# DiamondLightSource/volume-segmantics

Hardware: AMD Instinct MI355X
Metric: slices/sec fwd+bwd U-Net/ResNet-34 256x256 bf16 batch 32 (training step incl. loss, AdamW) (higher is better)
Workload: dtype bf16; 1 GPU; configs[1]: synthetic 256^3-style 1-ch slices, 2-class, U-Net/ResNet-34, batch 32 per GPU, train step (fwd + DiceLoss + bwd + AdamW + OneCycleLR); global_batch=32, slice=256x256, parallelism=dp1, master_weights=fp32

## Files before the change

volume-segmantics_amd/csrc/conv_common.h:

```cpp
#pragma once
#include <type_traits>

#include "common.h"

template <typename T> struct CT;
template <> struct CT<bf16_t> { static constexpr int CK = 32, EPS = 8; };
template <> struct CT<f16_t> { static constexpr int CK = 32, EPS = 8; };
template <> struct CT<float> { static constexpr int CK = 16, EPS = 4; };

template <typename T>
__device__ __forceinline__ float4 ld4_roundtrip(const float (&v)[4]) {
    if constexpr (sizeof(T) == 2) {
        const float a[4] = {v[0], v[1], v[2], v[3]};
        T t[4];
        for (int i = 0; i < 4; ++i) Elem<T>::st(t + i, a[i]);
        return make_float4(Elem<T>::ld(t), Elem<T>::ld(t + 1), Elem<T>::ld(t + 2), Elem<T>::ld(t + 3));
    } else
        return make_float4(v[0], v[1], v[2], v[3]);
}

template <typename T>
__device__ __forceinline__ void mma16(f32x4& acc, const uint4& a, const uint4& b) {
    if constexpr (std::is_same<T, f16_t>::value) {
        acc = __builtin_amdgcn_mfma_f32_16x16x32_f16(__builtin_bit_cast(f16x8, a), __builtin_bit_cast(f16x8, b), acc, 0, 0, 0);
    } else if constexpr (sizeof(T) == 2) {
        acc = __builtin_amdgcn_mfma_f32_16x16x32_bf16(__builtin_bit_cast(bf16x8, a), __builtin_bit_cast(bf16x8, b),
                                                      acc, 0, 0, 0);
    } else {
        const float4 fa = __builtin_bit_cast(float4, a), fb = __builtin_bit_cast(float4, b);
        acc = __builtin_amdgcn_mfma_f32_16x16x4f32(fa.x, fb.x, acc, 0, 0, 0);
        acc = __builtin_amdgcn_mfma_f32_16x16x4f32(fa.y, fb.y, acc, 0, 0, 0);
        acc = __builtin_amdgcn_mfma_f32_16x16x4f32(fa.z, fb.z, acc, 0, 0, 0);
        acc = __builtin_amdgcn_mfma_f32_16x16x4f32(fa.w, fb.w, acc, 0, 0, 0);
    }
}


template <typename T, int BN, int PT, int NW = 4>
__device__ __forceinline__ void conv_epilogue(const ConvParams& p, int tw_shift, int out_nchw, int n, int h0, int w0, int n0,
                                              int tile, f32x4 (&acc)[PT][BN / 16], char* smem) {
    constexpr int NJ = BN / 16;
    const int tid = threadIdx.x, lane = tid & 63, wave = tid >> 6;
    const int lq = lane >> 4, lr = lane & 15;
    const int TW = 1 << tw_shift;
    struct { int tw_shift, out_nchw; } g{tw_shift, out_nchw};
    const bool ragged = (p.Cout & 3) != 0 || g.out_nchw;
    if (p.stats_partial || p.stats_bins) {
        float* red = reinterpret_cast<float*>(smem);
        __syncthreads();
#pragma unroll
        for (int j = 0; j < NJ; ++j) {
            float s1[4] = {0.f, 0.f, 0.f, 0.f}, s2[4] = {0.f, 0.f, 0.f, 0.f};
#pragma unroll
            for (int i = 0; i < PT; ++i) {
                const int pl = wave * (PT * 16) + i * 16 + lr;
                const bool ok = h0 + (pl >> g.tw_shift) < p.Hout && w0 + (pl & (TW - 1)) < p.Wout;
#pragma unroll
                for (int r = 0; r < 4; ++r) {
                    const float x = ok ? acc[i][j][r] : 0.f;
                    s1[r] += x; s2[r] += x * x;
                }
            }
#pragma unroll
            for (int r = 0; r < 4; ++r) {
#pragma unroll
                for (int o = 1; o < 16; o <<= 1) { s1[r] += __shfl_xor(s1[r], o, 64); s2[r] += __shfl_xor(s2[r], o, 64); }
            }
            if (lr == 0) {
#pragma unroll
                for (int r = 0; r < 4; ++r) {
                    red[(wave * 2 + 0) * BN + j * 16 + lq * 4 + r] = s1[r];
                    red[(wave * 2 + 1) * BN + j * 16 + lq * 4 + r] = s2[r];
                }
            }
        }
        __syncthreads();
        if (tid < 2 * BN) {
            const int k = tid / BN, cc = tid % BN;
            if (n0 + cc < p.Cout) {
                float a = 0.f;
#pragma unroll
                for (int w = 0; w < NW; ++w) a += red[(w * 2 + k) * BN + cc];
                if (p.stats_bins)
                    atomicAdd(p.stats_bins + ((size_t)(tile & (p.stats_nb - 1)) * 2 + k) * p.Cout + n0 + cc,
                              (unsigned long long)__double2ll_rn((double)a * (k ? kStatScale2 : kStatScale1)));
                else
                    p.stats_partial[((size_t)tile * 2 + k) * p.Cout + n0 + cc] = a;
            }
        }
    }
    if (p.bz) {
        float* red = reinterpret_cast<float*>(smem);
        __syncthreads();
        typename Raw4<T>::type rv[PT][NJ], zq[PT][NJ], yq[PT][NJ];
        size_t off[PT][NJ];
        bool live[PT][NJ];
#pragma unroll
        for (int j = 0; j < NJ; ++j) {
            const int c = n0 + j * 16 + lq * 4;
#pragma unroll
            for (int i = 0; i < PT; ++i) {
                const int pl = wave * (PT * 16) + i * 16 + lr;
                const int ho = h0 + (pl >> g.tw_shift), wo = w0 + (pl & (TW - 1));
                live[i][j] = ho < p.Hout && wo < p.Wout && c < p.Cout;
                off[i][j] = (((size_t)n * p.Hout + ho) * p.Wout + wo) * p.Cout + c;
                rv[i][j] = zq[i][j] = yq[i][j] = typename Raw4<T>::type{};
                if (live[i][j]) {
                    if (p.residual) rv[i][j] = ld4raw((const T*)p.residual + off[i][j]);
                    zq[i][j] = ld4raw((const T*)p.bz + off[i][j]);
                    if (p.brelu && p.by) yq[i][j] = ld4raw((const T*)p.by + off[i][j]);
                }
            }
        }
#pragma unroll
        for (int j = 0; j < NJ; ++j) {
            const int c = n0 + j * 16 + lq * 4;
            float s1[4] = {0.f, 0.f, 0.f, 0.f}, s2[4] = {0.f, 0.f, 0.f, 0.f};
            float mu[4] = {0.f, 0.f, 0.f, 0.f}, is[4] = {0.f, 0.f, 0.f, 0.f}, ga[4] = {0.f, 0.f, 0.f, 0.f}, be[4] = {0.f, 0.f, 0.f, 0.f};
            if (c < p.Cout) {
                const float4 m4 = *reinterpret_cast<const float4*>(p.bmean + c), i4 = *reinterpret_cast<const float4*>(p.binvstd + c);
                mu[0] = m4.x; mu[1] = m4.y; mu[2] = m4.z; mu[3] = m4.w;
                is[0] = i4.x; is[1] = i4.y; is[2] = i4.z; is[3] = i4.w;
                if (p.brelu && !p.by) {
                    const float4 g4 = *reinterpret_cast<const float4*>(p.bgamma + c), b4 = *reinterpret_cast<const float4*>(p.bbeta + c);
                    ga[0] = is[0] * g4.x; ga[1] = is[1] * g4.y; ga[2] = is[2] * g4.z; ga[3] = is[3] * g4.w;
                    be[0] = b4.x; be[1] = b4.y; be[2] = b4.z; be[3] = b4.w;
                }
            }
#pragma unroll
            for (int i = 0; i < PT; ++i) {
                if (!live[i][j]) continue;
                const float4 r4 = unpack4(rv[i][j]), z4 = unpack4(zq[i][j]), y4 = unpack4(yq[i][j]);
                float v[4] = {acc[i][j][0] + r4.x, acc[i][j][1] + r4.y, acc[i][j][2] + r4.z, acc[i][j][3] + r4.w};
                const float zv[4] = {z4.x, z4.y, z4.z, z4.w};
                if (p.brelu) {
                    if (p.by) {
                        v[0] = y4.x > 0.f ? v[0] : 0.f; v[1] = y4.y > 0.f ? v[1] : 0.f;
                        v[2] = y4.z > 0.f ? v[2] : 0.f; v[3] = y4.w > 0.f ? v[3] : 0.f;
                    } else {
#pragma unroll
                        for (int r = 0; r < 4; ++r) v[r] = ((zv[r] - mu[r]) * ga[r] + be[r]) > 0.f ? v[r] : 0.f;
                    }
                }
                st4((T*)p.out + off[i][j], make_float4(v[0], v[1], v[2], v[3]));
                const float4 gq = ld4_roundtrip<T>(v);
                const float gv[4] = {gq.x, gq.y, gq.z, gq.w};
#pragma unroll
                for (int r = 0; r < 4; ++r) { s1[r] += gv[r]; s2[r] += gv[r] * (zv[r] - mu[r]) * is[r]; }
            }
#pragma unroll
            for (int r = 0; r < 4; ++r) {
#pragma unroll
                for (int o = 1; o < 16; o <<= 1) { s1[r] += __shfl_xor(s1[r], o, 64); s2[r] += __shfl_xor(s2[r], o, 64); }
            }
            if (lr == 0) {
#pragma unroll
                for (int r = 0; r < 4; ++r) {
                    red[(wave * 2 + 0) * BN + j * 16 + lq * 4 + r] = s1[r];
                    red[(wave * 2 + 1) * BN + j * 16 + lq * 4 + r] = s2[r];
                }
            }
        }
        __syncthreads();
        if (tid < 2 * BN) {
            const int k = tid / BN, cc = tid % BN;
            if (n0 + cc < p.Cout) {
                float a = 0.f;
#pragma unroll
                for (int w = 0; w < NW; ++w) a += red[(w * 2 + k) * BN + cc];
                p.bstats_partial[((size_t)tile * 2 + k) * p.Cout + n0 + cc] = a;
            }
        }
        return;
    }
    const int pool_c = p.pool0 ? (p.out1 ? p.split_c : p.Cout) : 0;
#pragma unroll
    for (int j = 0; j < NJ; ++j) {
        const int c = n0 + j * 16 + lq * 4;
        if (PT >= 2 && c < pool_c) {
            if constexpr (PT >= 2) {
#pragma unroll
                for (int ip = 0; ip < PT / 2; ++ip) {
                    float v[4];
#pragma unroll
                    for (int r = 0; r < 4; ++r) {
                        v[r] = acc[2 * ip][j][r] + acc[2 * ip + 1][j][r];
                        v[r] += __shfl_xor(v[r], 1, 64);
                    }
                    const int ho = h0 + wave * PT + 2 * ip, wo = w0 + lr;
                    if ((lr & 1) == 0 && ho < p.Hout && wo < p.Wout && c < p.Cout) {
                        const size_t o = (((size_t)n * (p.Hout >> 1) + (ho >> 1)) * (p.Wout >> 1) + (wo >> 1)) * pool_c + c;
                        st4((T*)p.out + o, make_float4(v[0], v[1], v[2], v[3]));
                    }
                }
            }
            continue;
        }
#pragma unroll
        for (int i = 0; i < PT; ++i) {
            const int pl = wave * (PT * 16) + i * 16 + lr;
            const int ho = h0 + (pl >> g.tw_shift), wo = w0 + (pl & (TW - 1));
            if (ho >= p.Hout || wo >= p.Wout || c >= p.Cout) continue;
            const size_t pix = ((size_t)n * p.Hout + ho) * p.Wout + wo;
            float v[4] = {acc[i][j][0], acc[i][j][1], acc[i][j][2], acc[i][j][3]};
            if (!ragged) {
                if (p.scale) {
                    const float4 sc = *reinterpret_cast<const float4*>(p.scale + c);
                    const float4 sh = *reinterpret_cast<const float4*>(p.shift + c);
                    v[0] = v[0] * sc.x + sh.x; v[1] = v[1] * sc.y + sh.y; v[2] = v[2] * sc.z + sh.z; v[3] = v[3] * sc.w + sh.w;
                } else if (p.shift) {
                    const float4 sh = *reinterpret_cast<const float4*>(p.shift + c);
                    v[0] += sh.x; v[1] += sh.y; v[2] += sh.z; v[3] += sh.w;
                }
                char* dst = (char*)p.out;
                int cd = c, cstride = p.Cout;
                if (p.out1) {
                    if (c >= p.split_c) { dst = (char*)p.out1; cd = c - p.split_c; cstride = p.Cout - p.split_c; }
                    else cstride = p.split_c;
                }
                const size_t o = pix * cstride + cd;
                if (p.residual && dst == (char*)p.out) {
                    const float4 rv = ld4((const T*)p.residual + o);
                    v[0] += rv.x; v[1] += rv.y; v[2] += rv.z; v[3] += rv.w;
                }
                if (p.relu == 1) { v[0] = fmaxf(v[0], 0.f); v[1] = fmaxf(v[1], 0.f); v[2] = fmaxf(v[2], 0.f); v[3] = fmaxf(v[3], 0.f); }
                else if (p.relu == 2) {
#pragma unroll
                    for (int r = 0; r < 4; ++r) v[r] = v[r] / (1.f + __expf(-v[r]));
                }
                if (p.out_f32) st4((float*)dst + o, make_float4(v[0], v[1], v[2], v[3]));
                else st4((T*)dst + o, make_float4(v[0], v[1], v[2], v[3]));
            } else {
                const int nv = min(4, p.Cout - c);
                for (int r = 0; r < nv; ++r) {
                    float x = v[r];
                    if (p.scale) x = x * p.scale[c + r] + p.shift[c + r];
                    else if (p.shift) x += p.shift[c + r];
                    if (p.residual) x += Elem<T>::ld((const T*)p.residual + pix * p.Cout + c + r);
                    if (p.relu == 1) x = fmaxf(x, 0.f);
                    else if (p.relu == 2) x = x / (1.f + __expf(-x));
                    if (g.out_nchw) ((float*)p.out)[(((size_t)n * p.Cout + c + r) * p.Hout + ho) * p.Wout + wo] = x;
                    else if (p.out_f32) ((float*)p.out)[pix * p.Cout + c + r] = x;
                    else Elem<T>::st((T*)p.out + pix * p.Cout + c + r, x);
                }
            }
        }
    }
}
```

volume-segmantics_amd/csrc/conv_ring.h:

```cpp
#pragma once
#include "conv_common.h"

namespace ring {

constexpr int kRow = 64;

__device__ __forceinline__ u32x4 make_srd(const void* base, unsigned bytes) {
    const unsigned long long a = (unsigned long long)base;
    u32x4 d;
    d.x = __builtin_amdgcn_readfirstlane((unsigned)a);
    d.y = __builtin_amdgcn_readfirstlane((unsigned)(a >> 32) & 0xffffu);
    d.z = __builtin_amdgcn_readfirstlane(bytes);
    d.w = 0x00020000u;
    return d;
}
template <int IMM>
__device__ __forceinline__ void dma16(const u32x4& srd, unsigned lds_base, int voff, int soff) {
    unsigned keep;
    asm volatile("s_mov_b32 %0, m0\n\ts_add_u32 m0, %1, %5\n\ts_nop 0\n\tbuffer_load_dwordx4 %2, %3, %4 offen lds\n\ts_mov_b32 m0, %0"
                 : "=&s"(keep) : "s"(lds_base), "v"(voff), "s"(srd), "s"(soff), "n"(IMM) : "memory", "scc");
}

template <typename A>
__device__ __forceinline__ A reload_first_kernarg() {
#if defined(__HIP_DEVICE_COMPILE__)
    const __attribute__((address_space(4))) A* pk = (const __attribute__((address_space(4))) A*)__builtin_amdgcn_kernarg_segment_ptr();
    asm volatile("" : "+s"(pk));
    return *pk;
#else
    return A{};
#endif
}

struct Geom {
    int tiles_h, tiles_w;
    int groups, ctiles;
    int xcs, xgn, ctl;
    unsigned ct_magic, ti_magic, tw_magic;
    int out_nchw;
    unsigned long long* probe;
};

constexpr int cdivc(int a, int b) { return (a + b - 1) / b; }
constexpr int minc(int a, int b) { return a < b ? a : b; }
template <int V> struct IC { static constexpr int value = V; };
template <int LO, int HI, typename F>
__device__ __forceinline__ void static_for(F&& f) {
    if constexpr (LO < HI) { f(IC<LO>{}); static_for<LO + 1, HI>(f); }
}

template <int BN, int PT, int NW, int TWS, int IMGS, int WPS, int PIN, bool NLOAD = false>
__global__ __launch_bounds__(NW * 64, WPS) void conv_ring_kernel(ConvParams p, Geom g) {
    typedef bf16_t T;
    constexpr int NT = NW * 64, NJ = BN / 16, BM = NW * PT * 16, TW = 1 << TWS, TH = BM / IMGS / TW;
    constexpr int PH = TH + 2, PW = TW + 2, PP = PH * PW, P = IMGS * PP;
    constexpr int PIT = cdivc(P * 4, NT);
    constexpr int WROWS = 9 * BN, TS = NT / 4 / BN;
    static_assert((NT / 4) % BN == 0, "cout tile must divide the rows of a piece pass");
    constexpr int WIT = cdivc(WROWS * 4, NT);
    constexpr int PATCH_B = PIT * NT * 16, WGT_B = WIT * NT * 16, STAGE_B = PATCH_B + WGT_B;
    constexpr int D = PIT + WIT, NG = 4, DG = cdivc(D, NG);
    static_assert(BM % (IMGS * TW) == 0 && TH * TW * IMGS == BM, "tile geometry");
    extern __shared__ __attribute__((aligned(16))) char smem[];
    const int tid = threadIdx.x, lane = tid & 63;
    const int wave = __builtin_amdgcn_readfirstlane(tid >> 6);
    const int lq = lane >> 4, lr = lane & 15;
    unsigned long long tprobe[5];
    if (g.probe) tprobe[0] = wall_clock64();

    const int xcd = blockIdx.x & 7, slot = blockIdx.x >> 3;
    const int xc = xcd & ((1 << g.xcs) - 1), xg = xcd >> g.xcs;
    const int gl = g.ctl == 1 ? slot : (int)__umulhi((unsigned)slot, g.ct_magic);
    const int ytile = xc * g.ctl + (slot - gl * g.ctl);
    const int grp = gl * g.xgn + xg;
    if (grp >= g.groups) return;
    int n, h0, w0, nimg;
    if constexpr (IMGS > 1) {
        n = grp * IMGS; h0 = 0; w0 = 0;
        nimg = min(IMGS, p.N - n);
    } else {
        const int tiles_img = g.tiles_h * g.tiles_w;
        n = tiles_img == 1 ? grp : (int)__umulhi((unsigned)grp, g.ti_magic);
        const int timg = grp - n * tiles_img;
        const int ty = g.tiles_w == 1 ? timg : (int)__umulhi((unsigned)timg, g.tw_magic);
        const int tx = timg - ty * g.tiles_w;
        h0 = ty * TH; w0 = tx * TW;
        nimg = 1;
    }
    const int n0 = ytile * BN;
    const int Cin = p.C0 + p.C1;
    const int ush = p.up0 ? 1 : 0;
    const bool stuffed = p.up0 == 2;
    const int H0 = p.Hin >> ush, W0 = p.Win >> ush;
    const u32x4 srd0 = make_srd((const T*)p.src0 + (size_t)n * H0 * W0 * p.C0, (unsigned)(nimg * H0 * W0 * p.C0 * 2));
    const u32x4 srd1 = make_srd((const T*)p.src1 + (size_t)n * p.Hin * p.Win * p.C1, p.src1 ? (unsigned)(nimg * p.Hin * p.Win * p.C1 * 2) : 0u);
    const u32x4 srdw = make_srd(p.w, (unsigned)(p.Cout * 9 * Cin * 2));
    const unsigned lds0 = (unsigned)(size_t)(__attribute__((address_space(3))) char*)smem;

    int poff0[PIT], poff1[PIT];
    unsigned nl_meta = 0;
#pragma unroll
    for (int i = 0; i < PIT; ++i) {
        const int it = tid + i * NT;
        const int pp = it >> 2;
        const int img = pp / PP, q = pp - img * PP;
        const int ph = q / PW, pw = q - ph * PW;
        const int seg = (it & 3) ^ ((pw >> 1) & 3);
        const int hi = h0 - 1 + ph, wi = w0 - 1 + pw;
        const bool ok = pp < P && img < nimg && hi >= 0 && hi < p.Hin && wi >= 0 && wi < p.Win;
        poff0[i] = (ok && !(stuffed && ((hi | wi) & 1))) ? (((img * H0 + (hi >> ush)) * W0 + (wi >> ush)) * p.C0 + seg * 8) * 2 : -1;
        poff1[i] = ok ? (((img * p.Hin + hi) * p.Win + wi) * p.C1 + seg * 8) * 2 : -1;
        if constexpr (NLOAD) {
            const bool mine = ok && ph >= 1 && ph <= TH && pw >= 1 && pw <= TW && !(ush && ((hi | wi) & 1));
            nl_meta |= ((unsigned)seg | (mine ? 4u : 0u)) << (4 * i);
        }
    }
    const int wrow0 = tid >> 2;
    const int wnr = wrow0 % BN, wtap0 = wrow0 / BN;
    const int wseg = (tid & 3) ^ ((wrow0 >> 1) & 3);
    int woff[WIT];
#pragma unroll
    for (int i = 0; i < WIT; ++i)
        woff[i] = (n0 + wnr < p.Cout && wtap0 + i * TS < 9) ? (((n0 + wnr) * 9 + wtap0 + i * TS) * Cin + wseg * 8) * 2 : -1;
    const bool ragged_c = ((p.C0 | p.C1) & 31) != 0;

    auto issue = [&](auto lo_, auto hi_, int c0, unsigned sb) {
        constexpr int LO = decltype(lo_)::value, HI = decltype(hi_)::value;
        const bool from0 = c0 < p.C0;
        const int cs = from0 ? p.C0 : p.C1;
        const int cb = from0 ? c0 : c0 - p.C0;
        const u32x4 srd = from0 ? srd0 : srd1;
        const int nseg = ragged_c ? (cs - cb) >> 3 : 4, nsegw = ragged_c ? (Cin - c0) >> 3 : 4;
        const unsigned wbase = sb + (unsigned)(wave * 1024);
        static_for<0, PIT>([&](auto ic) {
            constexpr int i = decltype(ic)::value;
            if constexpr (i >= LO && i < HI) {
                int off = from0 ? poff0[i] : poff1[i];
                if (ragged_c) {
                    const int it = tid + i * NT;
                    const int pp = it >> 2, q = pp % PP, pw = q % PW;
                    if (((it & 3) ^ ((pw >> 1) & 3)) >= nseg) off = -1;
                }
                dma16<i * NT * 16>(srd, wbase, off, cb * 2);
            }
        });
        static_for<0, WIT>([&](auto ic) {
            constexpr int i = decltype(ic)::value;
            if constexpr (PIT + i >= LO && PIT + i < HI) {
                int off = woff[i];
                if (ragged_c && wseg >= nsegw) off = -1;
                dma16<PATCH_B + i * NT * 16>(srdw, wbase, off, c0 * 2);
            }
        });
    };

    int xb[PT][3];
#pragma unroll
    for (int i = 0; i < PT; ++i) {
        const int pl = (tid >> 6) * (PT * 16) + i * 16 + lr;
        const int r = pl >> TWS, tw = pl & (TW - 1);
        const int img = r / TH, th = r - img * TH;
#pragma unroll
        for (int kw = 0; kw < 3; ++kw)
            xb[i][kw] = (img * PP + th * PW + tw + kw) * kRow + ((lq ^ (((tw + kw) >> 1) & 3)) << 4);
    }
    const int wb = PATCH_B + lr * kRow + ((lq ^ ((lr >> 1) & 3)) << 4);

    f32x4 acc[PT][NJ];
#pragma unroll
    for (int i = 0; i < PT; ++i)
#pragma unroll
        for (int j = 0; j < NJ; ++j) acc[i][j] = f32x4{0.f, 0.f, 0.f, 0.f};

    const int nch = (Cin + 31) >> 5;
    float* cst = reinterpret_cast<float*>(smem + 2 * STAGE_B);
    __amdgpu_buffer_rsrc_t sry = __builtin_amdgcn_make_buffer_rsrc(nullptr, 0, 0, 0x00020000);
    auto nl_stage = [&](char* st, int c0) {
        if (c0 >= p.C0) return;
        static_for<0, PIT>([&](auto ic) {
            constexpr int i = decltype(ic)::value;
            char* a = st + (tid + i * NT) * 16;
            const unsigned m = nl_meta >> (4 * i);
            const float* q = cst + c0 + (int)(m & 3u) * 8;
            float nm[8], na[8], nb[8];
#pragma unroll
            for (int h = 0; h < 2; ++h) {
                const float4 m4 = *reinterpret_cast<const float4*>(q + 4 * h), a4 = *reinterpret_cast<const float4*>(q + p.C0 + 4 * h),
                             b4 = *reinterpret_cast<const float4*>(q + 2 * p.C0 + 4 * h);
                nm[4 * h] = m4.x; nm[4 * h + 1] = m4.y; nm[4 * h + 2] = m4.z; nm[4 * h + 3] = m4.w;
                na[4 * h] = a4.x; na[4 * h + 1] = a4.y; na[4 * h + 2] = a4.z; na[4 * h + 3] = a4.w;
                nb[4 * h] = b4.x; nb[4 * h + 1] = b4.y; nb[4 * h + 2] = b4.z; nb[4 * h + 3] = b4.w;
            }
            const uint4 v = nl_apply8(*reinterpret_cast<const uint4*>(a), poff0[i] >= 0, nm, na, nb);
            *reinterpret_cast<uint4*>(a) = v;
            if (ytile == (c0 >> 5) % g.ctiles)
                __builtin_amdgcn_raw_buffer_store_b128(u32x4{v.x, v.y, v.z, v.w}, sry, (m & 4u) ? poff0[i] : (int)0x80000000, c0 * 2, 0);
        });
    };
    issue(IC<0>{}, IC<D>{}, 0, lds0);
    if (nch > 1) issue(IC<0>{}, IC<D>{}, 32, lds0 + STAGE_B);
    if constexpr (NLOAD) {
        sry = __builtin_amdgcn_make_buffer_rsrc((void*)((T*)p.nl_y + (size_t)n * H0 * W0 * p.C0), 0, nimg * H0 * W0 * p.C0 * 2, 0x00020000);
        const long long* bins = reinterpret_cast<const long long*>(p.nl_bins);
        const double rows = (double)p.nl_rows;
        for (int ch = tid; ch < p.C0; ch += NT) {
            long long sv = 0, qv = 0;
#pragma unroll 8
            for (int r = 0; r < p.nl_nb; ++r) { sv += bins[((size_t)r * 2 + 0) * p.C0 + ch]; qv += bins[((size_t)r * 2 + 1) * p.C0 + ch]; }
            const double mu = ((double)sv * (1.0 / kStatScale1)) / rows;
            double var = ((double)qv * (1.0 / kStatScale2)) / rows - mu * mu;
            if (var < 0.0) var = 0.0;
            const float is = (float)(1.0 / sqrt(var + (double)p.nl_eps));
            cst[ch] = (float)mu;
            cst[p.C0 + ch] = is * p.nl_gamma[ch];
            cst[2 * p.C0 + ch] = p.nl_beta[ch];
            if (blockIdx.x == 0) {
                p.nl_mean[ch] = (float)mu;
                p.nl_invstd[ch] = is;
                if (p.nl_rm) {
                    const double unbiased = p.nl_rows > 1 ? var * rows / (double)(p.nl_rows - 1) : var;
                    p.nl_rm[ch] = (float)((1.0 - p.nl_mom) * (double)p.nl_rm[ch] + p.nl_mom * mu);
                    p.nl_rv[ch] = (float)((1.0 - p.nl_mom) * (double)p.nl_rv[ch] + p.nl_mom * unbiased);
                }
            }
        }
        asm volatile("s_waitcnt vmcnt(0) lgkmcnt(0)" ::: "memory");
        __builtin_amdgcn_s_barrier();
        nl_stage(smem, 0);
        asm volatile("s_waitcnt lgkmcnt(0)" ::: "memory");
    } else if (nch > 1) {
        asm volatile("s_waitcnt vmcnt(%0)" ::"n"(D) : "memory");
    } else {
        asm volatile("s_waitcnt vmcnt(0)" ::: "memory");
    }
    __builtin_amdgcn_s_barrier();
    if (g.probe) tprobe[1] = tprobe[2] = wall_clock64();

    uint4 wf[3][NJ], xf[3][PT];
    auto read_frags = [&](const char* st, int tap, uint4 (&w)[NJ], uint4 (&x)[PT]) {
        const int kh = tap / 3, kw = tap % 3;
#pragma unroll
        for (int j = 0; j < NJ; ++j) w[j] = *reinterpret_cast<const uint4*>(st + wb + (tap * BN + j * 16) * kRow);
#pragma unroll
        for (int i = 0; i < PT; ++i) x[i] = *reinterpret_cast<const uint4*>(st + xb[i][kw] + kh * PW * kRow);
    };
    read_frags(smem, 0, wf[0], xf[0]);
    read_frags(smem, 1, wf[1], xf[1]);
    auto chunk_body = [&](int c, auto more_) {
        constexpr bool more = decltype(more_)::value != 0;
        const int s = c & 1;
        const char* cur = smem + s * STAGE_B;
        const char* nxt = smem + (s ^ 1) * STAGE_B;
        static_for<0, 9>([&](auto tc) {
            constexpr int t = decltype(tc)::value;
            if constexpr (t == 7 && more) {
                asm volatile("s_waitcnt vmcnt(0) lgkmcnt(0)" ::: "memory");
                if constexpr (NLOAD) {
                    nl_stage(const_cast<char*>(nxt), (c + 1) * 32);
                    asm volatile("s_waitcnt lgkmcnt(0)" ::: "memory");
                }
                __builtin_amdgcn_s_barrier();
            }
            if constexpr (t >= 7 && more) {
                if (c + 2 < nch) issue(IC<minc((t - 7) * DG, D)>{}, IC<minc((t - 6) * DG, D)>{}, (c + 2) * 32, lds0 + s * STAGE_B);
            } else if constexpr (t < NG - 2 && more) {
                if (c >= 1) issue(IC<minc((t + 2) * DG, D)>{}, IC<minc((t + 3) * DG, D)>{}, (c + 1) * 32, lds0 + (s ^ 1) * STAGE_B);
            }
            if constexpr (t + 2 < 9) read_frags(cur, t + 2, wf[(t + 2) % 3], xf[(t + 2) % 3]);
            else if constexpr (more) read_frags(nxt, t + 2 - 9, wf[(t + 2) % 3], xf[(t + 2) % 3]);
#pragma unroll
            for (int i = 0; i < PT; ++i)
#pragma unroll
                for (int j = 0; j < NJ; ++j) mma16<T>(acc[i][j], wf[t % 3][j], xf[t % 3][i]);
            if constexpr (PIN == 1) {
                if constexpr (t + 2 < 9 || more) __builtin_amdgcn_sched_group_barrier(0x100, NJ + PT, 0);
                __builtin_amdgcn_sched_group_barrier(0x008, NJ * PT, 0);
            } else if constexpr (PIN == 2) {
                constexpr int NR = (t + 2 < 9 || more) ? NJ + PT : 0, NM = NJ * PT;
                static_for<0, NR>([&](auto rc) {
                    constexpr int r = decltype(rc)::value;
                    __builtin_amdgcn_sched_group_barrier(0x100, 1, 0);
                    __builtin_amdgcn_sched_group_barrier(0x008, (NM * (r + 1)) / NR - (NM * r) / NR, 0);
                });
                if constexpr (NR == 0) __builtin_amdgcn_sched_group_barrier(0x008, NM, 0);
            }
        });
    };
    for (int c = 0; c + 1 < nch; ++c) chunk_body(c, IC<1>{});
    chunk_body(nch - 1, IC<0>{});

    if (g.probe) tprobe[3] = wall_clock64();
    const ConvParams pe = reload_first_kernarg<ConvParams>();
    if constexpr (IMGS > 1) {
        ConvParams q = pe;
        q.Hout = nimg * pe.Hout;
        conv_epilogue<T, BN, PT, NW>(q, TWS, g.out_nchw, grp, 0, 0, n0, grp, acc, smem);
    } else {
        conv_epilogue<T, BN, PT, NW>(pe, TWS, g.out_nchw, n, h0, w0, n0, grp, acc, smem);
    }
    if (g.probe) {
        __builtin_amdgcn_s_waitcnt(0);
        tprobe[4] = wall_clock64();
        if (tid == 0) {
            unsigned long long* o = g.probe + (size_t)blockIdx.x * 8;
            for (int i = 0; i < 5; ++i) o[i] = tprobe[i];
            unsigned hw, xcc;
            asm volatile("s_getreg_b32 %0, hwreg(HW_REG_HW_ID)" : "=s"(hw));
            asm volatile("s_getreg_b32 %0, hwreg(HW_REG_XCC_ID)" : "=s"(xcc));
            o[5] = hw; o[6] = xcc; o[7] = 0;
        }
    }
}

template <int BN, int PT, int NW, int TWS, int IMGS>
constexpr size_t ring_lds_bytes() {
    constexpr int NT = NW * 64, BM = NW * PT * 16, TW = 1 << TWS, TH = BM / IMGS / TW;
    constexpr int P = IMGS * (TH + 2) * (TW + 2);
    return 2 * (size_t)(cdivc(P * 4, NT) + cdivc(9 * BN * 4, NT)) * NT * 16;
}

template <int PT, int NW, int TWS, int IMGS>
inline bool ring_geom_ok(const ConvParams& p) {
    constexpr int BM = NW * PT * 16, TW = 1 << TWS, TH = BM / IMGS / TW;
    if (IMGS > 1) return p.Hout == TH && p.Wout == TW && p.N % IMGS == 0 && !(p.pool0);
    return true;
}

template <int BN, int PT, int NW, int TWS, int IMGS, int WPS, int PIN = 0, bool NLOAD = false>
int launch_ring(const ConvParams& p, int out_nchw, unsigned long long* probe, hipStream_t s) {
    static bool attr_set = false;
    auto kern = conv_ring_kernel<BN, PT, NW, TWS, IMGS, WPS, PIN, NLOAD>;
    constexpr size_t lds0 = ring_lds_bytes<BN, PT, NW, TWS, IMGS>();
    static_assert(lds0 <= 160 * 1024, "conv_ring: LDS ring too large");
    const size_t lds = lds0 + (NLOAD ? (size_t)3 * p.C0 * sizeof(float) : 0);
    VS_REQUIRE(lds <= 160 * 1024 && (!NLOAD || (p.nl_bins && !(p.C0 & 31) && p.up0 != 2)), "conv_ring: normalise-on-load needs C0 in whole chunks and room for its table");
    constexpr int BM = NW * PT * 16, TW = 1 << TWS, TH = BM / IMGS / TW;
    VS_REQUIRE(p.KH == 3 && p.KW == 3 && p.stride == 1 && p.pad == 1 && p.dil <= 1 && !p.gc, "conv_ring: stride-1 3x3 only");
    VS_REQUIRE((double)IMGS * p.Hin * p.Win * std::max(p.C0, p.C1) * 2.0 < 4.0e9 && (double)p.Cout * 9 * (p.C0 + p.C1) * 2.0 < 4.0e9,
               "conv_ring: image or weight tensor exceeds the 32-bit piece offsets");
    VS_REQUIRE((ring_geom_ok<PT, NW, TWS, IMGS>(p)), "conv_ring: geometry does not fit the tile");
    if (!attr_set) {
        VS_CHECK_HIP(hipFuncSetAttribute((const void*)kern, hipFuncAttributeMaxDynamicSharedMemorySize, 160 * 1024));
        attr_set = true;
    }
    Geom g{};
    g.tiles_h = IMGS > 1 ? 1 : cdiv(p.Hout, TH);
    g.tiles_w = IMGS > 1 ? 1 : cdiv(p.Wout, TW);
    g.groups = IMGS > 1 ? cdiv(p.N, IMGS) : p.N * g.tiles_h * g.tiles_w;
    g.ctiles = cdiv(p.Cout, BN);
    {
        const double wb = (double)p.Cout * 9 * (p.C0 + p.C1) * 2.0;
        const double ib = (double)p.N * ((double)(p.Hin >> (p.up0 ? 1 : 0)) * (p.Win >> (p.up0 ? 1 : 0)) * p.C0 + (double)p.Hin * p.Win * p.C1) * 2.0;
        int best = 0;
        double best_cost = 0;
        for (int xcs = 0; xcs <= 3; ++xcs) {
            const int xc = 1 << xcs;
            if (g.ctiles % xc) continue;
            const double cost = wb / xc + ib * xc / 8.0;
            if (xcs == 0 || !best_cost || cost < best_cost * 0.9) { best = xcs; best_cost = cost; }
        }
        g.xcs = best; g.xgn = 8 >> best; g.ctl = g.ctiles >> best;
    }
    g.ct_magic = 0xffffffffu / (unsigned)g.ctl + 1u;
    g.ti_magic = 0xffffffffu / (unsigned)(g.tiles_h * g.tiles_w) + 1u;
    g.tw_magic = 0xffffffffu / (unsigned)g.tiles_w + 1u;
    g.out_nchw = out_nchw;
    g.probe = probe;
    VS_REQUIRE(g.tiles_h * g.tiles_w < 65536 && p.N < 65536, "conv_ring: tile grid too large");
    const long nwg = (long)cdiv(g.groups, g.xgn) * g.ctl * 8;
    VS_REQUIRE(nwg < (1L << 31), "conv_ring: tile grid too large");
    hipLaunchKernelGGL(kern, dim3((unsigned)nwg), dim3(NW * 64), lds, s, p, g);
    VS_LAUNCH_CHECK();
    return VS_OK;
}

}
```

volume-segmantics_amd/csrc/conv_wgrad_ring.h:

```cpp
#pragma once
#include "conv_ring.h"

namespace ring {

__device__ __forceinline__ bool wg_assign(int xmode, int npairs, int nsplit, int ppx, int& pair, int& split) {
    if (xmode == 0) { pair = blockIdx.x; split = blockIdx.y; return true; }
    const int xcd = blockIdx.x & 7, j = blockIdx.x >> 3;
    if (xmode == 1) {
        const int sl = j / npairs;
        pair = j - sl * npairs;
        split = sl * 8 + xcd;
        return split < nsplit;
    }
    const int X = 8 / nsplit;
    split = xcd / X;
    pair = (xcd - split * X) * ppx + j;
    return j < ppx && pair < npairs;
}
inline unsigned wg_grid(int xmode, int npairs, int nsplit, int ppx) {
    return xmode == 0 ? 0u : (xmode == 1 ? 8u * ((nsplit + 7) / 8) * npairs : 8u * ppx);
}

struct WGeomR {
    int tiles_h, tiles_w, total_tiles, cchunks, nsplit;
    int xmode, npairs, ppx;
    unsigned tw_magic, th_magic;
    unsigned long long* probe;
};

__device__ __forceinline__ uint2 tr16(const char* p) {
    const short4v v = __builtin_amdgcn_ds_read_tr16_b64_v4i16((__attribute__((address_space(3))) short4v*)(p));
    return __builtin_bit_cast(uint2, v);
}

template <int MO, int TWS, int IMGS, int WPS>
__global__ __launch_bounds__(256, WPS) void conv_wgrad_ring_kernel(WgradParams p, WGeomR g) {
    constexpr int NTAPS = 9, BM = 128, KS = BM / 32, TW = 1 << TWS, TH = BM / IMGS / TW, PW = TW + 2, PH = TH + 2, PP = PH * PW, P = IMGS * PP;
    constexpr int kXP = 64;
    constexpr int BNO = 16 * MO, DYP = BNO * 2 < 64 ? 64 : BNO * 2, DSLOTS = DYP / 16, DSEG = BNO / 8, NSL = DYP / 32;
    constexpr int PIT = cdivc(P * 4, 256), DIT = BM * DSLOTS / 256;
    constexpr int PATCH_B = PIT * 256 * 16, DY_B = BM * DYP, STAGE_B = PATCH_B + DY_B;
    constexpr int D = PIT + DIT, NG = 4, DG = cdivc(D, NG);
    extern __shared__ __attribute__((aligned(16))) char smem[];
    const int tid = threadIdx.x, lane = tid & 63;
    const int wave = __builtin_amdgcn_readfirstlane(tid >> 6);
    const int lq = lane >> 4, lr = lane & 15;
    const int wc = wave & 1, wt = wave >> 1;
    unsigned long long tprobe[5];
    if (g.probe) tprobe[0] = wall_clock64();

    int pair, split;
    if (!wg_assign(g.xmode, g.npairs, g.nsplit, g.ppx, pair, split)) return;
    const int ct = pair / g.cchunks, cc = pair - ct * g.cchunks;
    const int co0 = ct * BNO, c0 = cc * 32;
    const int Cin = p.C0 + p.C1;
    const int per = (g.total_tiles + g.nsplit - 1) / g.nsplit;
    const int t0 = split * per, t1 = min(g.total_tiles, t0 + per);
    const int H0 = p.Hin >> p.up0, W0 = p.Win >> p.up0;
    const bool from0 = c0 < p.C0;
    const int cs = from0 ? p.C0 : p.C1;
    const int cb = from0 ? c0 : c0 - p.C0;
    const int sh = from0 ? p.up0 : 0;
    const int Hs = from0 ? H0 : p.Hin, Ws = from0 ? W0 : p.Win;
    const u32x4 srdx = make_srd(from0 ? p.src0 : p.src1, (unsigned)(p.N * Hs * Ws * cs * 2));
    const u32x4 srdd = make_srd(p.dy, (unsigned)(p.N * p.Hout * p.Wout * p.Cout * 2));
    const unsigned lds0 = (unsigned)(size_t)(__attribute__((address_space(3))) char*)smem;

    int pph[PIT], ppw[PIT], pco[PIT];
#pragma unroll
    for (int i = 0; i < PIT; ++i) {
        const int it = tid + i * 256;
        const int pp = it >> 2, sp = it & 3;
        const int img = pp / PP, q0 = pp - img * PP;
        const int ph = q0 / PW, pw = q0 - ph * PW;
        const int seg = ((((sp >> 1) ^ (pw >> 3)) & 1) << 1) | (sp & 1);
        pph[i] = (img << 8) | ph; ppw[i] = pw;
        pco[i] = (pp < P && cb + seg * 8 < cs) ? (cb + seg * 8) * 2 : -1;
    }
    int drow[DIT], dco[DIT];
#pragma unroll
    for (int i = 0; i < DIT; ++i) {
        const int it = tid + i * 256;
        const int r = it / DSLOTS, sp = it % DSLOTS;
        const int dgk = NSL == 4 ? (((r >> 1) & 1) | (((r >> 3) & 1) << 1)) : ((r >> 3) & 1);
        const int dseg = ((((sp >> 1) ^ dgk) & (NSL - 1)) << 1) | (sp & 1);
        drow[i] = r;
        dco[i] = (dseg < DSEG && co0 + dseg * 8 < p.Cout) ? (co0 + dseg * 8) * 2 : -1;
    }
    auto issue = [&](auto lo_, auto hi_, int tile, unsigned sb) {
        constexpr int LO = decltype(lo_)::value, HI = decltype(hi_)::value;
        int n, h0, w0;
        if constexpr (IMGS > 1) {
            n = tile * IMGS; h0 = 0; w0 = 0;
        } else {
            const int q = g.tiles_w == 1 ? tile : (int)__umulhi((unsigned)tile, g.tw_magic);
            const int tx = tile - q * g.tiles_w;
            n = g.tiles_h == 1 ? q : (int)__umulhi((unsigned)q, g.th_magic);
            const int ty = q - n * g.tiles_h;
            h0 = ty * TH; w0 = tx * TW;
        }
        const unsigned wbase = sb + (unsigned)(wave * 1024);
        static_for<0, PIT>([&](auto ic) {
            constexpr int i = decltype(ic)::value;
            if constexpr (i >= LO && i < HI) {
                const int ni = n + (pph[i] >> 8);
                const int hi = h0 - 1 + (pph[i] & 255), wi = w0 - 1 + ppw[i];
                const bool ok = pco[i] >= 0 && ni < p.N && hi >= 0 && hi < p.Hin && wi >= 0 && wi < p.Win;
                const int off = ((ni * Hs + (hi >> sh)) * Ws + (wi >> sh)) * cs * 2 + pco[i];
                dma16<i * 4096>(srdx, wbase, ok ? off : -1, 0);
            }
        });
        static_for<0, DIT>([&](auto ic) {
            constexpr int i = decltype(ic)::value;
            if constexpr (PIT + i >= LO && PIT + i < HI) {
                const int rr = drow[i] >> TWS;
                const int ni = n + rr / TH;
                const int ho = h0 + rr % TH, wo = w0 + (drow[i] & (TW - 1));
                const bool ok = dco[i] >= 0 && ni < p.N && ho < p.Hout && wo < p.Wout;
                const int off = ((ni * p.Hout + ho) * p.Wout + wo) * p.Cout * 2 + dco[i];
                dma16<PATCH_B + i * 4096>(srdd, wbase, ok ? off : -1, 0);
            }
        });
    };

    int a_addr[2][MO], x_addr[2][3];
#pragma unroll
    for (int h = 0; h < 2; ++h) {
        const int px = 8 * lq + (lr >> 2) + 4 * h;
        const int gk = NSL == 4 ? (((px >> 1) & 1) | (((px >> 3) & 1) << 1)) : ((px >> 3) & 1);
#pragma unroll
        for (int m = 0; m < MO; ++m) a_addr[h][m] = PATCH_B + ((px * DYP + (gk << 5) + (lr & 3) * 8) ^ (m << 5));
        const int row0 = (px >> TWS) * PW, col0 = px & (TW - 1);
#pragma unroll
        for (int kw = 0; kw < 3; ++kw)
            x_addr[h][kw] = (row0 + col0 + kw) * kXP + ((wc ^ ((col0 + kw) >> 3)) & 1) * 32 + (lr & 3) * 8;
    }
    auto ks_off = [](int ks) { const int r = ks * (32 >> TWS); return ((r / TH) * PP + (r % TH) * PW) * kXP; };

    f32x4 acc[5][MO];
#pragma unroll
    for (int t = 0; t < 5; ++t)
#pragma unroll
        for (int m = 0; m < MO; ++m) acc[t][m] = f32x4{0.f, 0.f, 0.f, 0.f};

    if (t0 < t1) {
        issue(IC<0>{}, IC<D>{}, t0, lds0);
        if (t0 + 1 < t1) {
            issue(IC<0>{}, IC<D>{}, t0 + 1, lds0 + STAGE_B);
            asm volatile("s_waitcnt vmcnt(%0)" ::"n"(D) : "memory");
        } else {
            asm volatile("s_waitcnt vmcnt(0)" ::: "memory");
        }
    }
    __builtin_amdgcn_s_barrier();
    if (g.probe) tprobe[1] = tprobe[2] = wall_clock64();

    auto run = [&](auto t0_, auto ntp_) {
        constexpr int T0 = decltype(t0_)::value, NTP = decltype(ntp_)::value, NS = KS * NTP;
        uint4 af[2][MO], bf[4];
        auto read_b = [&](const char* st, int s, uint4& b) {
            const int ks = s / NTP, t = T0 + s % NTP, kh = t / 3, kw = t % 3;
            const uint2 lo = tr16(st + x_addr[0][kw] + kh * PW * kXP + ks_off(ks));
            const uint2 hi = tr16(st + x_addr[1][kw] + kh * PW * kXP + ks_off(ks));
            b = make_uint4(lo.x, lo.y, hi.x, hi.y);
        };
        auto read_a = [&](const char* st, int ks, uint4 (&a)[MO]) {
#pragma unroll
            for (int m = 0; m < MO; ++m) {
                const uint2 lo = tr16(st + a_addr[0][m] + ks * 32 * DYP);
                const uint2 hi = tr16(st + a_addr[1][m] + ks * 32 * DYP);
                a[m] = make_uint4(lo.x, lo.y, hi.x, hi.y);
            }
        };
        auto reads_for = [&](const char* st, auto s2_) {
            constexpr int s2 = decltype(s2_)::value;
            if constexpr (s2 % NTP == 0) read_a(st, s2 / NTP, af[(s2 / NTP) & 1]);
            read_b(st, s2, bf[s2 % 4]);
        };
        auto tile_body = [&](int tile, auto more_) {
            constexpr bool more = decltype(more_)::value != 0;
            const int sidx = (tile - t0) & 1;
            const char* cur = smem + sidx * STAGE_B;
            const char* nxt = smem + (sidx ^ 1) * STAGE_B;
            static_for<0, NS>([&](auto sc) {
                constexpr int s = decltype(sc)::value;
                if constexpr (s == NS - 2 && more) {
                    asm volatile("s_waitcnt vmcnt(0) lgkmcnt(0)" ::: "memory");
                    __builtin_amdgcn_s_barrier();
                }
                if constexpr (s >= NS - 2 && more) {
                    if (tile + 2 < t1) issue(IC<minc((s - (NS - 2)) * DG, D)>{}, IC<minc((s - (NS - 2) + 1) * DG, D)>{}, tile + 2, lds0 + sidx * STAGE_B);
                } else if constexpr (s < NG - 2 && more) {
                    if (tile > t0) issue(IC<minc((s + 2) * DG, D)>{}, IC<minc((s + 3) * DG, D)>{}, tile + 1, lds0 + (sidx ^ 1) * STAGE_B);
                }
                constexpr int s2 = s + 2;
                constexpr bool has_reads = s2 < NS || more;
                if constexpr (s2 < NS) reads_for(cur, IC<s2>{});
                else if constexpr (more) reads_for(nxt, IC<s2 - NS>{});
                constexpr int ks = s / NTP, tt = s % NTP;
#pragma unroll
                for (int m = 0; m < MO; ++m)
                    acc[tt][m] = __builtin_amdgcn_mfma_f32_16x16x32_bf16(__builtin_bit_cast(bf16x8, af[ks & 1][m]),
                                                                         __builtin_bit_cast(bf16x8, bf[s % 4]), acc[tt][m], 0, 0, 0);
                constexpr int NR = has_reads ? 2 + (((s2 % NS) % NTP == 0) ? 2 * MO : 0) : 0;
                if constexpr (NR > 0) __builtin_amdgcn_sched_group_barrier(0x100, NR, 0);
                __builtin_amdgcn_sched_group_barrier(0x008, MO, 0);
            });
        };
        if (t0 < t1) {
            static_assert(NS % 4 == 0 && KS % 2 == 0, "fragment ring indices must run on across tiles");
            reads_for(smem, IC<0>{});
            reads_for(smem, IC<1>{});
            for (int tile = t0; tile + 1 < t1; ++tile) tile_body(tile, IC<1>{});
            tile_body(t1 - 1, IC<0>{});
        }
    };
    if (wt == 0) run(IC<0>{}, IC<5>{});
    else run(IC<5>{}, IC<4>{});

    if (g.probe) tprobe[3] = wall_clock64();
    float* out = p.partials + (size_t)split * p.Cout * NTAPS * Cin;
    const int ci = c0 + wc * 16 + lr;
    if (ci < Cin) {
#pragma unroll
        for (int tt = 0; tt < 5; ++tt) {
            const int t = wt * 5 + tt;
            if (t >= NTAPS) continue;
#pragma unroll
            for (int m = 0; m < MO; ++m)
#pragma unroll
                for (int r = 0; r < 4; ++r) {
                    const int co = co0 + m * 16 + lq * 4 + r;
                    if (co < p.Cout) out[((size_t)co * NTAPS + t) * Cin + ci] = acc[tt][m][r];
                }
        }
    }
    if (g.probe) {
        __builtin_amdgcn_s_waitcnt(0);
        tprobe[4] = wall_clock64();
        if (tid == 0) {
            unsigned long long* o = g.probe + ((size_t)blockIdx.y * gridDim.x + blockIdx.x) * 8;
            for (int i = 0; i < 5; ++i) o[i] = tprobe[i];
            unsigned hw, xcc;
            asm volatile("s_getreg_b32 %0, hwreg(HW_REG_HW_ID)" : "=s"(hw));
            asm volatile("s_getreg_b32 %0, hwreg(HW_REG_XCC_ID)" : "=s"(xcc));
            o[5] = hw; o[6] = xcc; o[7] = 0;
        }
    }
}

template <int MO, int TWS, int IMGS>
constexpr size_t wgrad_ring_lds() {
    constexpr int BNO = 16 * MO, DYP = BNO * 2 < 64 ? 64 : BNO * 2, TW = 1 << TWS, TH = 128 / IMGS / TW;
    return 2 * (size_t)(cdivc(IMGS * (TH + 2) * (TW + 2) * 4, 256) * 256 * 16 + 128 * DYP);
}

}
```

Baseline: 7269 slices/s.

## Batch epilogue global loads before use and preload kernargs into scalar registers

The conv epilogue now issues all residual, bz and by loads, plus the scale and shift vectors, up front. Out-of-range lanes use clamped addresses so the loads are unconditional, and an empty asm barrier forces them to land together instead of in serialised per-element chunks. BN mean, invstd and gamma/beta are fetched once per lane and broadcast through LDS, and the ragged/non-ragged output path is split at compile time. The conv and wgrad ring kernels force kernel arguments into SGPRs early and reload the epilogue ConvParams during the last chunk so that load overlaps compute. The cost is higher register pressure, extra LDS use and some redundant loads from clamped addresses.

```diff
diff --git a/volume-segmantics_amd/csrc/conv_common.h b/volume-segmantics_amd/csrc/conv_common.h
--- a/volume-segmantics_amd/csrc/conv_common.h
+++ b/volume-segmantics_amd/csrc/conv_common.h
@@ -18,6 +18,10 @@
     } else
         return make_float4(v[0], v[1], v[2], v[3]);
 }
+
+__device__ __forceinline__ void landed(const uint2& v) { asm volatile("" ::"v"(v.x), "v"(v.y)); }
+__device__ __forceinline__ void landed(const float4& v) { asm volatile("" ::"v"(v.x), "v"(v.y), "v"(v.z), "v"(v.w)); }
+__device__ __forceinline__ void landed(const f16raw4& v) { landed(v.u); }
 
 template <typename T>
 __device__ __forceinline__ void mma16(f32x4& acc, const uint4& a, const uint4& b) {
@@ -45,6 +49,7 @@
     const int TW = 1 << tw_shift;
     struct { int tw_shift, out_nchw; } g{tw_shift, out_nchw};
     const bool ragged = (p.Cout & 3) != 0 || g.out_nchw;
+    __builtin_amdgcn_s_waitcnt(0x0f70);
     if (p.stats_partial || p.stats_bins) {
         float* red = reinterpret_cast<float*>(smem);
         __syncthreads();
@@ -91,7 +96,15 @@
     }
     if (p.bz) {
         float* red = reinterpret_cast<float*>(smem);
+        float* par = red + (NW * 2 + wave * 4) * BN;
         __syncthreads();
+        const bool affine = p.brelu && !p.by;
+        float pm = 0.f, pi = 0.f, pg = 0.f, pb = 0.f;
+        if (BN == 64 || lane < BN) {
+            const int cp = min(n0 + lane, p.Cout - 1);
+            pm = p.bmean[cp]; pi = p.binvstd[cp];
+            if (affine) { pg = p.bgamma[cp]; pb = p.bbeta[cp]; }
+        }
         typename Raw4<T>::type rv[PT][NJ], zq[PT][NJ], yq[PT][NJ];
         size_t off[PT][NJ];
         bool live[PT][NJ];
@@ -104,28 +117,36 @@
                 const int ho = h0 + (pl >> g.tw_shift), wo = w0 + (pl & (TW - 1));
                 live[i][j] = ho < p.Hout && wo < p.Wout && c < p.Cout;
                 off[i][j] = (((size_t)n * p.Hout + ho) * p.Wout + wo) * p.Cout + c;
-                rv[i][j] = zq[i][j] = yq[i][j] = typename Raw4<T>::type{};
-                if (live[i][j]) {
-                    if (p.residual) rv[i][j] = ld4raw((const T*)p.residual + off[i][j]);
-                    zq[i][j] = ld4raw((const T*)p.bz + off[i][j]);
-                    if (p.brelu && p.by) yq[i][j] = ld4raw((const T*)p.by + off[i][j]);
-                }
-            }
-        }
-#pragma unroll
-        for (int j = 0; j < NJ; ++j) {
-            const int c = n0 + j * 16 + lq * 4;
+                const size_t lo = live[i][j] ? off[i][j] : (size_t)0;
+                rv[i][j] = yq[i][j] = typename Raw4<T>::type{};
+                if (p.residual) rv[i][j] = ld4raw((const T*)p.residual + lo);
+                zq[i][j] = ld4raw((const T*)p.bz + lo);
+                if (p.brelu && p.by) yq[i][j] = ld4raw((const T*)p.by + lo);
+            }
+        }
+#pragma unroll
+        for (int j = 0; j < NJ; ++j)
+#pragma unroll
+            for (int i = 0; i < PT; ++i) {
+                landed(zq[i][j]);
+                if (p.residual) landed(rv[i][j]);
+                if (p.brelu && p.by) landed(yq[i][j]);
+            }
+        if (BN == 64 || lane < BN) {
+            par[lane] = pm; par[BN + lane] = pi;
+            if (affine) { par[2 * BN + lane] = pi * pg; par[3 * BN + lane] = pb; }
+        }
+        __builtin_amdgcn_wave_barrier();
+#pragma unroll
+        for (int j = 0; j < NJ; ++j) {
             float s1[4] = {0.f, 0.f, 0.f, 0.f}, s2[4] = {0.f, 0.f, 0.f, 0.f};
-            float mu[4] = {0.f, 0.f, 0.f, 0.f}, is[4] = {0.f, 0.f, 0.f, 0.f}, ga[4] = {0.f, 0.f, 0.f, 0.f}, be[4] = {0.f, 0.f, 0.f, 0.f};
-            if (c < p.Cout) {
-                const float4 m4 = *reinterpret_cast<const float4*>(p.bmean + c), i4 = *reinterpret_cast<const float4*>(p.binvstd + c);
-                mu[0] = m4.x; mu[1] = m4.y; mu[2] = m4.z; mu[3] = m4.w;
-                is[0] = i4.x; is[1] = i4.y; is[2] = i4.z; is[3] = i4.w;
-                if (p.brelu && !p.by) {
-                    const float4 g4 = *reinterpret_cast<const float4*>(p.bgamma + c), b4 = *reinterpret_cast<const float4*>(p.bbeta + c);
-                    ga[0] = is[0] * g4.x; ga[1] = is[1] * g4.y; ga[2] = is[2] * g4.z; ga[3] = is[3] * g4.w;
-                    be[0] = b4.x; be[1] = b4.y; be[2] = b4.z; be[3] = b4.w;
-                }
+            float ga[4] = {0.f, 0.f, 0.f, 0.f}, be[4] = {0.f, 0.f, 0.f, 0.f};
+            const float4 m4 = *reinterpret_cast<const float4*>(par + j * 16 + lq * 4), i4 = *reinterpret_cast<const float4*>(par + BN + j * 16 + lq * 4);
+            const float mu[4] = {m4.x, m4.y, m4.z, m4.w}, is[4] = {i4.x, i4.y, i4.z, i4.w};
+            if (affine) {
+                const float4 g4 = *reinterpret_cast<const float4*>(par + 2 * BN + j * 16 + lq * 4), b4 = *reinterpret_cast<const float4*>(par + 3 * BN + j * 16 + lq * 4);
+                ga[0] = g4.x; ga[1] = g4.y; ga[2] = g4.z; ga[3] = g4.w;
+                be[0] = b4.x; be[1] = b4.y; be[2] = b4.z; be[3] = b4.w;
             }
 #pragma unroll
             for (int i = 0; i < PT; ++i) {
@@ -174,76 +195,113 @@
         return;
     }
     const int pool_c = p.pool0 ? (p.out1 ? p.split_c : p.Cout) : 0;
-#pragma unroll
-    for (int j = 0; j < NJ; ++j) {
-        const int c = n0 + j * 16 + lq * 4;
-        if (PT >= 2 && c < pool_c) {
-            if constexpr (PT >= 2) {
-#pragma unroll
-                for (int ip = 0; ip < PT / 2; ++ip) {
-                    float v[4];
-#pragma unroll
-                    for (int r = 0; r < 4; ++r) {
-                        v[r] = acc[2 * ip][j][r] + acc[2 * ip + 1][j][r];
-                        v[r] += __shfl_xor(v[r], 1, 64);
-                    }
-                    const int ho = h0 + wave * PT + 2 * ip, wo = w0 + lr;
-                    if ((lr & 1) == 0 && ho < p.Hout && wo < p.Wout && c < p.Cout) {
-                        const size_t o = (((size_t)n * (p.Hout >> 1) + (ho >> 1)) * (p.Wout >> 1) + (wo >> 1)) * pool_c + c;
-                        st4((T*)p.out + o, make_float4(v[0], v[1], v[2], v[3]));
-                    }
-                }
-            }
-            continue;
-        }
-#pragma unroll
-        for (int i = 0; i < PT; ++i) {
-            const int pl = wave * (PT * 16) + i * 16 + lr;
-            const int ho = h0 + (pl >> g.tw_shift), wo = w0 + (pl & (TW - 1));
-            if (ho >= p.Hout || wo >= p.Wout || c >= p.Cout) continue;
-            const size_t pix = ((size_t)n * p.Hout + ho) * p.Wout + wo;
-            float v[4] = {acc[i][j][0], acc[i][j][1], acc[i][j][2], acc[i][j][3]};
-            if (!ragged) {
-                if (p.scale) {
-                    const float4 sc = *reinterpret_cast<const float4*>(p.scale + c);
-                    const float4 sh = *reinterpret_cast<const float4*>(p.shift + c);
-                    v[0] = v[0] * sc.x + sh.x; v[1] = v[1] * sc.y + sh.y; v[2] = v[2] * sc.z + sh.z; v[3] = v[3] * sc.w + sh.w;
-                } else if (p.shift) {
-                    const float4 sh = *reinterpret_cast<const float4*>(p.shift + c);
-                    v[0] += sh.x; v[1] += sh.y; v[2] += sh.z; v[3] += sh.w;
-                }
-                char* dst = (char*)p.out;
-                int cd = c, cstride = p.Cout;
-                if (p.out1) {
-                    if (c >= p.split_c) { dst = (char*)p.out1; cd = c - p.split_c; cstride = p.Cout - p.split_c; }
-                    else cstride = p.split_c;
-                }
-                const size_t o = pix * cstride + cd;
-                if (p.residual && dst == (char*)p.out) {
-                    const float4 rv = ld4((const T*)p.residual + o);
-                    v[0] += rv.x; v[1] += rv.y; v[2] += rv.z; v[3] += rv.w;
-                }
-                if (p.relu == 1) { v[0] = fmaxf(v[0], 0.f); v[1] = fmaxf(v[1], 0.f); v[2] = fmaxf(v[2], 0.f); v[3] = fmaxf(v[3], 0.f); }
-                else if (p.relu == 2) {
-#pragma unroll
-                    for (int r = 0; r < 4; ++r) v[r] = v[r] / (1.f + __expf(-v[r]));
-                }
-                if (p.out_f32) st4((float*)dst + o, make_float4(v[0], v[1], v[2], v[3]));
-                else st4((T*)dst + o, make_float4(v[0], v[1], v[2], v[3]));
-            } else {
-                const int nv = min(4, p.Cout - c);
-                for (int r = 0; r < nv; ++r) {
-                    float x = v[r];
-                    if (p.scale) x = x * p.scale[c + r] + p.shift[c + r];
-                    else if (p.shift) x += p.shift[c + r];
-                    if (p.residual) x += Elem<T>::ld((const T*)p.residual + pix * p.Cout + c + r);
-                    if (p.relu == 1) x = fmaxf(x, 0.f);
-                    else if (p.relu == 2) x = x / (1.f + __expf(-x));
-                    if (g.out_nchw) ((float*)p.out)[(((size_t)n * p.Cout + c + r) * p.Hout + ho) * p.Wout + wo] = x;
-                    else if (p.out_f32) ((float*)p.out)[pix * p.Cout + c + r] = x;
-                    else Elem<T>::st((T*)p.out + pix * p.Cout + c + r, x);
-                }
-            }
+    float4 sc4[NJ], sh4[NJ];
+    typename Raw4<T>::type rq[PT][NJ];
+    if (!ragged && (p.scale || p.shift || p.residual)) {
+        const float* scp = p.scale ? p.scale : (const float*)p.w;
+        const float* shp = p.shift ? p.shift : (const float*)p.w;
+        const T* rp = p.residual ? (const T*)p.residual : (const T*)p.w;
+#pragma unroll
+        for (int j = 0; j < NJ; ++j) {
+            const int c = n0 + j * 16 + lq * 4;
+            const int cl = c < p.Cout ? c : 0;
+            sc4[j] = *reinterpret_cast<const float4*>(scp + (p.scale ? cl : 0));
+            sh4[j] = *reinterpret_cast<const float4*>(shp + (p.shift ? cl : 0));
+        }
+#pragma unroll
+        for (int j = 0; j < NJ; ++j) {
+            const int c = n0 + j * 16 + lq * 4;
+#pragma unroll
+            for (int i = 0; i < PT; ++i) {
+                const int pl = wave * (PT * 16) + i * 16 + lr;
+                const int ho = h0 + (pl >> g.tw_shift), wo = w0 + (pl & (TW - 1));
+                const bool to_out = !p.out1 || c < p.split_c;
+                const bool use = p.residual && ho < p.Hout && wo < p.Wout && c < p.Cout && !(PT >= 2 && c < pool_c) && to_out;
+                const size_t o = (((size_t)n * p.Hout + ho) * p.Wout + wo) * (p.out1 ? p.split_c : p.Cout) + c;
+                rq[i][j] = ld4raw(rp + (use ? o : (size_t)0));
+            }
+        }
+#pragma unroll
+        for (int j = 0; j < NJ; ++j) {
+            landed(sc4[j]); landed(sh4[j]);
+#pragma unroll
+            for (int i = 0; i < PT; ++i) landed(rq[i][j]);
         }
     }
+    auto outputs = [&](auto ragged_) {
+        constexpr bool kRagged = decltype(ragged_)::value;
+#pragma unroll
+        for (int j = 0; j < NJ; ++j) {
+            const int c = n0 + j * 16 + lq * 4;
+            if (PT >= 2 && c < pool_c) {
+                if constexpr (PT >= 2) {
+#pragma unroll
+                    for (int ip = 0; ip < PT / 2; ++ip) {
+                        float v[4];
+#pragma unroll
+                        for (int r = 0; r < 4; ++r) {
+                            v[r] = acc[2 * ip][j][r] + acc[2 * ip + 1][j][r];
+                            v[r] += __shfl_xor(v[r], 1, 64);
+                        }
+                        const int ho = h0 + wave * PT + 2 * ip, wo = w0 + lr;
+                        if ((lr & 1) == 0 && ho < p.Hout && wo < p.Wout && c < p.Cout) {
+                            const size_t o = (((size_t)n * (p.Hout >> 1) + (ho >> 1)) * (p.Wout >> 1) + (wo >> 1)) * pool_c + c;
+                            st4((T*)p.out + o, make_float4(v[0], v[1], v[2], v[3]));
+                        }
+                    }
+                }
+                continue;
+            }
+#pragma unroll
+            for (int i = 0; i < PT; ++i) {
+                const int pl = wave * (PT * 16) + i * 16 + lr;
+                const int ho = h0 + (pl >> g.tw_shift), wo = w0 + (pl & (TW - 1));
+                if (ho >= p.Hout || wo >= p.Wout || c >= p.Cout) continue;
+                const size_t pix = ((size_t)n * p.Hout + ho) * p.Wout + wo;
+                float v[4] = {acc[i][j][0], acc[i][j][1], acc[i][j][2], acc[i][j][3]};
+                if constexpr (!kRagged) {
+                    if (p.scale) {
+                        const float4 sc = sc4[j], sh = sh4[j];
+                        v[0] = v[0] * sc.x + sh.x; v[1] = v[1] * sc.y + sh.y; v[2] = v[2] * sc.z + sh.z; v[3] = v[3] * sc.w + sh.w;
+                    } else if (p.shift) {
+                        const float4 sh = sh4[j];
+                        v[0] += sh.x; v[1] += sh.y; v[2] += sh.z; v[3] += sh.w;
+                    }
+                    char* dst = (char*)p.out;
+                    int cd = c, cstride = p.Cout;
+                    if (p.out1) {
+                        if (c >= p.split_c) { dst = (char*)p.out1; cd = c - p.split_c; cstride = p.Cout - p.split_c; }
+                        else cstride = p.split_c;
+                    }
+                    const size_t o = pix * cstride + cd;
+                    if (p.residual && dst == (char*)p.out) {
+                        const float4 rv = unpack4(rq[i][j]);
+                        v[0] += rv.x; v[1] += rv.y; v[2] += rv.z; v[3] += rv.w;
+                    }
+                    if (p.relu == 1) { v[0] = fmaxf(v[0], 0.f); v[1] = fmaxf(v[1], 0.f); v[2] = fmaxf(v[2], 0.f); v[3] = fmaxf(v[3], 0.f); }
+                    else if (p.relu == 2) {
+#pragma unroll
+                        for (int r = 0; r < 4; ++r) v[r] = v[r] / (1.f + __expf(-v[r]));
+                    }
+                    if (p.out_f32) st4((float*)dst + o, make_float4(v[0], v[1], v[2], v[3]));
+                    else st4((T*)dst + o, make_float4(v[0], v[1], v[2], v[3]));
+                } else {
+                    const int nv = min(4, p.Cout - c);
+                    for (int r = 0; r < nv; ++r) {
+                        float x = v[r];
+                        if (p.scale) x = x * p.scale[c + r] + p.shift[c + r];
+                        else if (p.shift) x += p.shift[c + r];
+                        if (p.residual) x += Elem<T>::ld((const T*)p.residual + pix * p.Cout + c + r);
+                        if (p.relu == 1) x = fmaxf(x, 0.f);
+                        else if (p.relu == 2) x = x / (1.f + __expf(-x));
+                        if (g.out_nchw) ((float*)p.out)[(((size_t)n * p.Cout + c + r) * p.Hout + ho) * p.Wout + wo] = x;
+                        else if (p.out_f32) ((float*)p.out)[pix * p.Cout + c + r] = x;
+                        else Elem<T>::st((T*)p.out + pix * p.Cout + c + r, x);
+                    }
+                }
+            }
+        }
+    };
+    if (ragged) outputs(std::true_type{});
+    else outputs(std::false_type{});
 }
diff --git a/volume-segmantics_amd/csrc/conv_ring.h b/volume-segmantics_amd/csrc/conv_ring.h
--- a/volume-segmantics_amd/csrc/conv_ring.h
+++ b/volume-segmantics_amd/csrc/conv_ring.h
@@ -65,6 +65,9 @@
     const int tid = threadIdx.x, lane = tid & 63;
     const int wave = __builtin_amdgcn_readfirstlane(tid >> 6);
     const int lq = lane >> 4, lr = lane & 15;
+    asm volatile("" ::"s"(p.src0), "s"(p.src1), "s"(p.w), "s"(p.C0), "s"(p.C1), "s"(p.up0), "s"(p.N), "s"(p.Hin), "s"(p.Win), "s"(p.Cout),
+                 "s"(g.tiles_h), "s"(g.tiles_w), "s"(g.groups), "s"(g.xcs), "s"(g.xgn), "s"(g.ctl), "s"(g.ct_magic), "s"(g.ti_magic),
+                 "s"(g.tw_magic), "s"(g.probe));
     unsigned long long tprobe[5];
     if (g.probe) tprobe[0] = wall_clock64();
 
@@ -246,8 +249,10 @@
     };
     read_frags(smem, 0, wf[0], xf[0]);
     read_frags(smem, 1, wf[1], xf[1]);
+    ConvParams pe;
     auto chunk_body = [&](int c, auto more_) {
         constexpr bool more = decltype(more_)::value != 0;
+        if constexpr (!more) pe = reload_first_kernarg<ConvParams>();
         const int s = c & 1;
         const char* cur = smem + s * STAGE_B;
         const char* nxt = smem + (s ^ 1) * STAGE_B;
@@ -290,7 +295,6 @@
     chunk_body(nch - 1, IC<0>{});
 
     if (g.probe) tprobe[3] = wall_clock64();
-    const ConvParams pe = reload_first_kernarg<ConvParams>();
     if constexpr (IMGS > 1) {
         ConvParams q = pe;
         q.Hout = nimg * pe.Hout;
diff --git a/volume-segmantics_amd/csrc/conv_wgrad_ring.h b/volume-segmantics_amd/csrc/conv_wgrad_ring.h
--- a/volume-segmantics_amd/csrc/conv_wgrad_ring.h
+++ b/volume-segmantics_amd/csrc/conv_wgrad_ring.h
@@ -46,6 +46,9 @@
     const int wave = __builtin_amdgcn_readfirstlane(tid >> 6);
     const int lq = lane >> 4, lr = lane & 15;
     const int wc = wave & 1, wt = wave >> 1;
+    asm volatile("" ::"s"(p.src0), "s"(p.src1), "s"(p.dy), "s"(p.C0), "s"(p.C1), "s"(p.up0), "s"(p.N), "s"(p.Hin), "s"(p.Win), "s"(p.Hout),
+                 "s"(p.Wout), "s"(p.Cout), "s"(g.tiles_h), "s"(g.tiles_w), "s"(g.total_tiles), "s"(g.cchunks), "s"(g.nsplit), "s"(g.xmode),
+                 "s"(g.npairs), "s"(g.ppx), "s"(g.tw_magic), "s"(g.th_magic), "s"(g.probe));
     unsigned long long tprobe[5];
     if (g.probe) tprobe[0] = wall_clock64();
 
```

New measurement: 7413 slices/s, median of 6. +2.0%, better.
